# lgleznah/mort

Measured on AMD Instinct MI355X. Metric: Msamples/sec (width x height x spp/s), Scene 1 1200x675, higher is better.
Workload: dtype f32; 1 GPU; Scene 1 (random-spheres cover) 1200x675, 500 spp nominal = 484 effective, depth 20, megakernel, seed 69420, host LCG scene; mode=mega, partition=rows/8 interleaved over 1 rank(s)

## Files before the change

mort_amd/csrc/hip/mega_bvh.h:

```cpp
#ifndef MORT_MEGA_BVH_H
#define MORT_MEGA_BVH_H

#include "dev_render.h"


struct FastArgs {
    RenderArgs r;
    const unsigned char *hot_src;
    uint32_t hot_bytes;
    uint32_t off_nodes4, off_leafrecs, off_lambert, off_metal, off_diel, off_dlight, off_iso, off_solid, off_checker;
    uint32_t off_tstack;
    int node_first, node_count;
    unsigned int *next_q;
    int tiles_x, tiles_total;
    uint32_t off_stack;
    int stack_lds_depth;
    const unsigned *tile_order;
    int gen_tiles;
    int spread_shift;
    unsigned *tile_cost;
    int th_s, th_l, t_keep;
    int sub;
    float *vaccum;
    float4 *deep;
    int prio_tiles, prio_lanes;
    int drain_rounds;
    int tile_key_sum;
    const unsigned *prio_dev;
    int heavy_mod, heavy_num, heavy_cap;
    int lane_cap;
    unsigned long long *wave_log;
};

#ifdef MORT_BVH_PRIVATE_ARGS
#define MORT_BVH_ARG_NAME fa_byval
#else
#define MORT_BVH_ARG_NAME
#endif
#ifdef MORT_BVH_NO_PIN
#define BU_I(x) (x)
#define BU_U(x) (x)
#define BU_F(x) (x)
#define BU_P(x) (x)
#else
#define BU_I(x) uni_i(x)
#define BU_U(x) uni_u(x)
#define BU_F(x) uni_f(x)
#define BU_P(x) uni_p(x)
#endif
__device__ __forceinline__ int uni_i(int x) { return __builtin_amdgcn_readfirstlane(x); }
__device__ __forceinline__ uint32_t uni_u(uint32_t x) { return (uint32_t)__builtin_amdgcn_readfirstlane((int)x); }
__device__ __forceinline__ float uni_f(float x) { return __int_as_float(__builtin_amdgcn_readfirstlane(__float_as_int(x))); }
template <typename T> __device__ __forceinline__ T *uni_p(T *p) {
    const unsigned long long v = (unsigned long long)p;
    const uint32_t lo = uni_u((uint32_t)v), hi = uni_u((uint32_t)(v >> 32));
    return (T *)(((unsigned long long)hi << 32) | (unsigned long long)lo);
}

enum { ST_T = 0, ST_L = 1, ST_S = 2, ST_DONE = 3 };
enum { FL_TIE = 1, FL_REF = 2, FL_MASK = 3 };
#define FL_SIGNS(ox, oy, oz) (int)(((ox) << 8) | ((oy) << 16) | ((oz) << 24))
#ifdef MORT_REGION_MARKS
#define REGION(name) asm volatile("; REGION " name)
#else
#define REGION(name) do { } while (0)
#endif

DEV bool own_inv_ok(float v) { const float a = mort_fabsf(v); return a > 1e-15f && a < 1e15f; }
struct V3Ret { float x, y, z; };
__device__ __attribute__((noinline)) V3Ret texture_value_uv(const DScene *sc, uint32_t tex, float nx, float ny, float nz, float px, float py, float pz) {
    float u, v;
    sphere_uv(mk(nx, ny, nz), u, v);
    const V3 c = texture_value(*sc, tex, u, v, mk(px, py, pz));
    V3Ret r; r.x = c.x; r.y = c.y; r.z = c.z;
    return r;
}

struct RefHit { int best; float closest; };
__device__ __attribute__((noinline)) RefHit reference_walk(const DBvhNode *nodes, int node_first, int node_end, const DSphere *spheres,
                                                           float ox, float oy, float oz, float dx, float dy, float dz, float tm, float ray_a) {
    Ray ray; ray.o = mk(ox, oy, oz); ray.d = mk(dx, dy, dz); ray.tm = tm;
    float closest = __builtin_inff();
    int best = -1;
    const double dix = 1.0 / (double)ray.d.x, diy = 1.0 / (double)ray.d.y, diz = 1.0 / (double)ray.d.z;
    int n = node_first;
    while (n < node_end) {
        const DBvhNode nd = nodes[n];
        const int skip = (int)(nd.skip & 0x7fffffffu);
        if (!slab_exact(nd, ray.o.x, ray.o.y, ray.o.z, dix, diy, diz, closest)) { n = skip; continue; }
        if (!(nd.skip >> 31)) { n = n + 1; continue; }
        const uint32_t pa = nd.prims & 0x7fffu, pb = (nd.prims >> 16) & 0x7fffu;
        for (int k = 0; k < 2; k++) {
            const uint32_t p = k ? pb : pa;
            if (k == 1 && pb == pa) break;
            float t;
            if (sphere_hit_t(spheres[p], ray, ray_a, 0.001f, closest, t)) { closest = t; best = (int)p; }
        }
        n = skip;
    }
    RefHit h; h.best = best; h.closest = closest;
    return h;
}

DEV float sphere_hit_root(const DSphere &s, const Ray &r, float a, float t_min, float t_max) {
    const V3 oc = vsub(r.o, sphere_center(s, r.tm));
    const float half_b = vdot(oc, r.d);
    const float c = vlen2(oc) - s.radius * s.radius;
    const float discriminant = half_b * half_b - a * c;
    if (discriminant < 0) return -1.0f;
    const float sqrtd = mort_sqrtf(discriminant);
    float root = (-half_b - sqrtd) / a;
    if (root < t_min || t_max < root) {
        root = (-half_b + sqrtd) / a;
        if (root < t_min || t_max < root) return -1.0f;
    }
    return root;
}

struct OwnRay { float ix, iy, iz, mx, my, mz, band, invlen; };

DEV bool own_prune(float xmin, float xmax, float ymin, float ymax, float zmin, float zmax, float e, const OwnRay &r, float closest, float &te_out) {
    const float px0 = __builtin_fmaf(xmin, r.ix, -r.mx), px1 = __builtin_fmaf(xmax, r.ix, -r.mx);
    const float py0 = __builtin_fmaf(ymin, r.iy, -r.my), py1 = __builtin_fmaf(ymax, r.iy, -r.my);
    const float pz0 = __builtin_fmaf(zmin, r.iz, -r.mz), pz1 = __builtin_fmaf(zmax, r.iz, -r.mz);
    const float te = __builtin_fmaxf(__builtin_fmaxf(__builtin_fminf(px0, px1), __builtin_fminf(py0, py1)),
                                     __builtin_fmaxf(__builtin_fminf(pz0, pz1), 0.001f));
    const float tx = __builtin_fminf(__builtin_fminf(__builtin_fmaxf(px0, px1), __builtin_fmaxf(py0, py1)), __builtin_fmaxf(pz0, pz1));
    const float tau = __builtin_fmaf(__builtin_fmaxf(mort_fabsf(te), mort_fabsf(tx)), 9.5367431640625e-07f, r.band);
    const float key = __builtin_fmaf(te, 0.992f, -__builtin_fmaf(e, r.invlen, tau));
    te_out = te;
    return (tx - te < -tau) || (key > closest);
}

DEV bool own_prune_ordered(float xn, float xf, float yn, float yf, float zn, float zf, float e, const OwnRay &r, float closest, float &te_out) {
    const float pxn = __builtin_fmaf(xn, r.ix, -r.mx), pxf = __builtin_fmaf(xf, r.ix, -r.mx);
    const float pyn = __builtin_fmaf(yn, r.iy, -r.my), pyf = __builtin_fmaf(yf, r.iy, -r.my);
    const float pzn = __builtin_fmaf(zn, r.iz, -r.mz), pzf = __builtin_fmaf(zf, r.iz, -r.mz);
    const float te = __builtin_fmaxf(__builtin_fmaxf(pxn, pyn), __builtin_fmaxf(pzn, 0.001f));
    const float tx = __builtin_fminf(__builtin_fminf(pxf, pyf), pzf);
    const float tau = __builtin_fmaf(__builtin_fmaxf(mort_fabsf(te), mort_fabsf(tx)), 9.5367431640625e-07f, r.band);
    const float key = __builtin_fmaf(te, 0.992f, -__builtin_fmaf(e, r.invlen, tau));
    te_out = te;
    return (tx - te < -tau) || (key > closest);
}
DEV uint32_t own_sign_offset(float inv) { return (__builtin_bit_cast(uint32_t, inv) >> 27) & 16u; }

typedef float v2f_t __attribute__((ext_vector_type(2)));
DEV void own_prune2(v2f_t xmin, v2f_t xmax, v2f_t ymin, v2f_t ymax, v2f_t zmin, v2f_t zmax, v2f_t e, const OwnRay &r, float closest,
                    float &te_a, float &te_b, bool &skip_a, bool &skip_b) {
    const v2f_t ix = {r.ix, r.ix}, iy = {r.iy, r.iy}, iz = {r.iz, r.iz};
    const v2f_t nmx = {-r.mx, -r.mx}, nmy = {-r.my, -r.my}, nmz = {-r.mz, -r.mz};
    const v2f_t px0 = __builtin_elementwise_fma(xmin, ix, nmx), px1 = __builtin_elementwise_fma(xmax, ix, nmx);
    const v2f_t py0 = __builtin_elementwise_fma(ymin, iy, nmy), py1 = __builtin_elementwise_fma(ymax, iy, nmy);
    const v2f_t pz0 = __builtin_elementwise_fma(zmin, iz, nmz), pz1 = __builtin_elementwise_fma(zmax, iz, nmz);
    v2f_t te, tx;
    te.x = __builtin_fmaxf(__builtin_fmaxf(__builtin_fminf(px0.x, px1.x), __builtin_fminf(py0.x, py1.x)), __builtin_fmaxf(__builtin_fminf(pz0.x, pz1.x), 0.001f));
    te.y = __builtin_fmaxf(__builtin_fmaxf(__builtin_fminf(px0.y, px1.y), __builtin_fminf(py0.y, py1.y)), __builtin_fmaxf(__builtin_fminf(pz0.y, pz1.y), 0.001f));
    tx.x = __builtin_fminf(__builtin_fminf(__builtin_fmaxf(px0.x, px1.x), __builtin_fmaxf(py0.x, py1.x)), __builtin_fmaxf(pz0.x, pz1.x));
    tx.y = __builtin_fminf(__builtin_fminf(__builtin_fmaxf(px0.y, px1.y), __builtin_fmaxf(py0.y, py1.y)), __builtin_fmaxf(pz0.y, pz1.y));
    v2f_t am;
    am.x = __builtin_fmaxf(mort_fabsf(te.x), mort_fabsf(tx.x)); am.y = __builtin_fmaxf(mort_fabsf(te.y), mort_fabsf(tx.y));
    const v2f_t c20 = {9.5367431640625e-07f, 9.5367431640625e-07f}, band = {r.band, r.band}, il = {r.invlen, r.invlen}, c992 = {0.992f, 0.992f};
    const v2f_t tau = __builtin_elementwise_fma(am, c20, band);
    const v2f_t key = __builtin_elementwise_fma(te, c992, -__builtin_elementwise_fma(e, il, tau));
    const v2f_t gap = tx - te;
    te_a = te.x; te_b = te.y;
    skip_a = (gap.x < -tau.x) || (key.x > closest);
    skip_b = (gap.y < -tau.y) || (key.y > closest);
}

// ... 164 lines not shown
            pf.lofs = qx + qly * a.width;
            pf.got = SUB ? 1 + (qly - rly * fa.sub) : 1;
            done = true;
        }
    }
    if (pf.got) {
        const mort_rng_state st = a.states[pf.lofs];
        pf.d = st.d; pf.v0 = st.v[0]; pf.v1 = st.v[1]; pf.v2 = st.v[2]; pf.v3 = st.v[3]; pf.v4 = st.v[4];
    }
    return pf;
}

template <int BLOCK, bool PROBE, bool DRAIN = false, bool SUB = false>
__global__ void __launch_bounds__(BLOCK, BLOCK == 1024 ? 4 : (DRAIN && BLOCK < 768) ? (BLOCK + 255) / 256 : MORT_MIN_WAVES) mega_bvh_kernel(const FastArgs MORT_BVH_ARG_NAME) {
    extern __shared__ __attribute__((aligned(16))) unsigned char lds[];
    __shared__ CamView s_cam;
#ifdef MORT_BVH_PRIVATE_ARGS
    const FastArgs *const fap = &fa_byval;
    const FastArgs &s_fa = fa_byval;
#else
    __shared__ FastArgs s_fa;
    const FastArgs *const fap = (const FastArgs *)__builtin_amdgcn_kernarg_segment_ptr();
    {
        const uint32_t *src = (const uint32_t *)fap;
        uint32_t *dst = (uint32_t *)&s_fa;
        for (uint32_t i = threadIdx.x; i < (uint32_t)(sizeof(FastArgs) / 4); i += BLOCK) dst[i] = src[i];
    }
#endif
    {
        const uint4 *src = (const uint4 *)fap->hot_src;
        uint4 *dst = (uint4 *)lds;
        const uint32_t n16 = fap->hot_bytes >> 4;
        for (uint32_t i = threadIdx.x; i < n16; i += BLOCK) dst[i] = src[i];
    }
    __syncthreads();
    if (threadIdx.x == 0) cam_view_fill(s_cam, s_fa.r);
    __syncthreads();
    const FastArgs &L = s_fa;
    static_assert(sizeof(DNode4) == 16 * MORT_NODE4_PIECES && sizeof(DLeaf2) == 16 * MORT_LEAF2_PIECES, "record strides");
    const float4 *nodes4 = (const float4 *)(lds + BU_U(L.off_nodes4));
    const float4 *leafrecs = (const float4 *)(lds + BU_U(L.off_leafrecs));
    unsigned short *const ts_base = (unsigned short *)(lds + BU_U(L.off_tstack)) + threadIdx.x;
#define TS_AT(ptr) (*(ptr))
    const DLambert *lambert = (const DLambert *)(lds + BU_U(L.off_lambert));
    const DMetal *metal = (const DMetal *)(lds + BU_U(L.off_metal));
    const DDielectric *dielectric = (const DDielectric *)(lds + BU_U(L.off_diel));
    const DLambert *dlight = (const DLambert *)(lds + BU_U(L.off_dlight));
    const DLambert *isotropic = (const DLambert *)(lds + BU_U(L.off_iso));
    const DSolid *solid = (const DSolid *)(lds + BU_U(L.off_solid));
    const DChecker *checker = (const DChecker *)(lds + BU_U(L.off_checker));

    const int node_first = BU_I(L.node_first), node_end = node_first + BU_I(L.node_count);
    const int th_s = BU_I(L.th_s), th_l = BU_I(L.th_l), t_keep = BU_I(L.t_keep);
    const int sqrt_spp = BU_I(L.r.sqrt_spp), bounce_limit = BU_I(L.r.bounce_limit);
    const float bg_x = BU_F(L.r.background.x), bg_y = BU_F(L.r.background.y), bg_z = BU_F(L.r.background.z);
    const int spp = sqrt_spp * sqrt_spp;
    const unsigned total_q = (unsigned)BU_I(L.tiles_total) * 64u;

    int state = ((int)(threadIdx.x & 63u) < BU_I(L.lane_cap)) ? ST_S : ST_DONE, kind = K_NEWPIX;
    int xy = 0, lofs = 0;
    Rng rng; rng.d = rng.v0 = rng.v1 = rng.v2 = rng.v3 = rng.v4 = 0; rng.draws = 0;
    V3 pixel_color = mk(0, 0, 0);
    int s_ij = 0, iter = 0;
    uint32_t segments = 0;
    Ray ray; ray.o = mk(0, 0, 0); ray.d = mk(0, 0, 1); ray.tm = 0;
    float ray_time0 = 0;
    OwnRay orr; orr.ix = orr.iy = orr.iz = 1; orr.mx = orr.my = orr.mz = 0; orr.band = 0; orr.invlen = 1;
    float ray_a = 1, closest = 0;
    int best = -1;
    uint32_t node = 0;
    unsigned short *spa = ts_base;
    int flags = 0;
    float4 *stack_deep = BU_P(L.deep) + ((size_t)blockIdx.x * BLOCK + threadIdx.x);
    const size_t deep_stride = (size_t)gridDim.x * BLOCK;
    unsigned long long ident_mask = 0ull;
    float4 *stack_lds = (float4 *)(lds + BU_U(L.off_stack));
    const int DL = BU_I(L.stack_lds_depth);
#ifdef MORT_PROFILE_STATES
    unsigned long long *const counters_p = fap->r.counters;
    unsigned long long prof[6] = {0, 0, 0, 0, 0, 0};
    unsigned long long prof_truns = 0;
    unsigned long long profc[8] = {0, 0, 0, 0, 0, 0, 0, 0};
    unsigned long long ps0 = 0, ps1;
#define PROFS0() do { ps0 = __builtin_readcyclecounter(); } while (0)
#define PROFS(i) do { ps1 = __builtin_readcyclecounter(); profc[i] += ps1 - ps0; ps0 = ps1; } while (0)
    unsigned long long pt0 = __builtin_readcyclecounter(), pt1;
    const unsigned long long prof_r0 = __builtin_amdgcn_s_memrealtime();
#define PROF(i, lanes) do { prof[2 * (i)] += 1; prof[2 * (i) + 1] += (unsigned long long)(lanes); } while (0)
    unsigned long long profb[12] = {0, 0, 0, 0, 0, 0, 0, 0, 0, 0, 0, 0};
#ifdef MORT_PROFILE_FINE
#define PROFB(i) do { } while (0)
    unsigned long long proff[12] = {0, 0, 0, 0, 0, 0, 0, 0, 0, 0, 0, 0};
#define PROFF(i) do { ps1 = __builtin_readcyclecounter(); proff[i] += ps1 - ps0; profc[4] += ps1 - ps0; ps0 = ps1; } while (0)
#else
#define PROFF(i) do { } while (0)
#define PROFB(i) do { const unsigned long long m_ = __ballot(1); if ((int)(threadIdx.x & 63) == __ffsll((long long)m_) - 1) { \
        atomicAdd(&counters_p[18 + 2 * (i)], 1ull); atomicAdd(&counters_p[19 + 2 * (i)], (unsigned long long)__popcll(m_)); } } while (0)
#endif
#define PROFC(i) do { pt1 = __builtin_readcyclecounter(); profc[i] += pt1 - pt0; pt0 = pt1; } while (0)
#else
#define PROF(i, lanes) do { } while (0)
#define PROFB(i) do { } while (0)
#define PROFF(i) do { } while (0)
#define PROFC(i) do { } while (0)
#define PROFS0() do { } while (0)
#define PROFS(i) do { } while (0)
#endif

    int leader = -1;
    const bool drain_rounds = DRAIN && BU_I(L.drain_rounds) == 1;
    const bool live_thresholds = BU_I(L.drain_rounds) == 3;
    bool running = true;
    while (running) {
      int nS = 0;
      for (;;) {
        const unsigned long long mT = __ballot(state == ST_T);
        const unsigned long long mL = __ballot(state == ST_L);
        const unsigned long long mS = __ballot(state == ST_S);
        if ((mT | mL | mS) == 0ull) { running = false; break; }
        const int nT = __popcll(mT), nL = __popcll(mL);
        nS = __popcll(mS);
        int pick;
        int e_s = th_s, e_l = th_l;
        if (live_thresholds) { const int live = nT + nL + nS; e_s = (th_s * live + 63) >> 6; e_l = (th_l * live + 63) >> 6; }
        if (nS >= e_s) pick = ST_S;
        else if (nL >= e_l) pick = ST_L;
        else if (nT > 0) pick = ST_T;
        else pick = (nL >= nS) ? ST_L : ST_S;
        if (DRAIN && leader >= 0) {
            if (drain_rounds) pick = nT > 0 ? ST_T : nL > 0 ? ST_L : ST_S;
            else { const int ls = __builtin_amdgcn_readlane(state, leader); if (ls <= ST_S) pick = ls; }
        }
        PROFC(3);

                REGION("T");
        if (pick != ST_T && pick != ST_L) break;
        if (pick == ST_T) {
            int keep;
#ifdef MORT_PROFILE_STATES
            prof_truns++;
#endif
            do {
#pragma unroll
                for (int rep = 0; rep < MORT_T_UNROLL; rep++) {
                PROF(0, __popcll(__ballot(state == ST_T)));
                if (state == ST_T) {
                    const float4 *np = nodes4 + node;
                    float t0, t1, t2, t3;
#ifdef MORT_BVH_PACKED_FMA
                    const float4 bx0 = np[MORT_NODE4_X], bx1 = np[MORT_NODE4_X + 1], by0 = np[MORT_NODE4_Y], by1 = np[MORT_NODE4_Y + 1];
                    const float4 bz0 = np[MORT_NODE4_Z], bz1 = np[MORT_NODE4_Z + 1], be = np[MORT_NODE4_E];
                    const uint4 ch = ((const uint4 *)np)[MORT_NODE4_CHILD];
                    bool m0, m1, m2, m3;
                    own_prune2(v2f_t{bx0.x, bx0.y}, v2f_t{bx1.x, bx1.y}, v2f_t{by0.x, by0.y}, v2f_t{by1.x, by1.y}, v2f_t{bz0.x, bz0.y}, v2f_t{bz1.x, bz1.y}, v2f_t{be.x, be.y}, orr, closest, t0, t1, m0, m1);
                    own_prune2(v2f_t{bx0.z, bx0.w}, v2f_t{bx1.z, bx1.w}, v2f_t{by0.z, by0.w}, v2f_t{by1.z, by1.w}, v2f_t{bz0.z, bz0.w}, v2f_t{bz1.z, bz1.w}, v2f_t{be.z, be.w}, orr, closest, t2, t3, m2, m3);
                    m2 = m2 || ch.z == 0xffffu; m3 = m3 || ch.w == 0xffffu;
#else
                    const unsigned char *nb = (const unsigned char *)np;
                    const float4 *ax = (const float4 *)(nb + (((uint32_t)flags >> 8) & 0xffu)) + MORT_NODE4_X;
                    const float4 *ay = (const float4 *)(nb + (((uint32_t)flags >> 16) & 0xffu)) + MORT_NODE4_Y;
                    const float4 *az = (const float4 *)(nb + ((uint32_t)flags >> 24)) + MORT_NODE4_Z;
                    const float4 xn = ax[0], xf = ax[1], yn = ay[0], yf = ay[1], zn = az[0], zf = az[1], be = np[MORT_NODE4_E];
                    const uint4 ch = ((const uint4 *)np)[MORT_NODE4_CHILD];
                    const bool m0 = own_prune_ordered(xn.x, xf.x, yn.x, yf.x, zn.x, zf.x, be.x, orr, closest, t0);
                    const bool m1 = own_prune_ordered(xn.y, xf.y, yn.y, yf.y, zn.y, zf.y, be.y, orr, closest, t1);
                    const bool m2 = own_prune_ordered(xn.z, xf.z, yn.z, yf.z, zn.z, zf.z, be.z, orr, closest, t2) || ch.z == 0xffffu;
                    const bool m3 = own_prune_ordered(xn.w, xf.w, yn.w, yf.w, zn.w, zf.w, be.w, orr, closest, t3) || ch.w == 0xffffu;
#endif
                    uint32_t k0 = m0 ? 0xffffffffu : ((__float_as_uint(t0) & 0xffff0000u) | ch.x);
                    uint32_t k1 = m1 ? 0xffffffffu : ((__float_as_uint(t1) & 0xffff0000u) | ch.y);
                    uint32_t k2 = m2 ? 0xffffffffu : ((__float_as_uint(t2) & 0xffff0000u) | ch.z);
                    uint32_t k3 = m3 ? 0xffffffffu : ((__float_as_uint(t3) & 0xffff0000u) | ch.w);
#define MORT_CSWAP(a, b) do { const uint32_t lo_ = a < b ? a : b, hi_ = a < b ? b : a; a = lo_; b = hi_; } while (0)
                    MORT_CSWAP(k0, k1); MORT_CSWAP(k2, k3); MORT_CSWAP(k0, k2); MORT_CSWAP(k1, k3); MORT_CSWAP(k1, k2);
#undef MORT_CSWAP
#ifdef MORT_BVH_PUSH_BRANCHFREE
                    TS_AT(spa) = (unsigned short)k3; spa += (k3 != 0xffffffffu) ? BLOCK : 0;
                    TS_AT(spa) = (unsigned short)k2; spa += (k2 != 0xffffffffu) ? BLOCK : 0;
                    TS_AT(spa) = (unsigned short)k1; spa += (k1 != 0xffffffffu) ? BLOCK : 0;
#else
                    if (k3 != 0xffffffffu) { TS_AT(spa) = (unsigned short)k3; spa += BLOCK; }
                    if (k2 != 0xffffffffu) { TS_AT(spa) = (unsigned short)k2; spa += BLOCK; }
                    if (k1 != 0xffffffffu) { TS_AT(spa) = (unsigned short)k1; spa += BLOCK; }
#endif
                    uint32_t next = k0;
                    const bool none = k0 == 0xffffffffu;
                    const bool have = !none || spa != ts_base;
                    if (none && spa != ts_base) { spa -= BLOCK; next = TS_AT(spa); }
                    if (!have) { state = ST_S; kind = K_SHADE; }
                    else { node = next & 0x7fffu; if (next & 0x8000u) state = ST_L; }
                }
                }
                keep = __popcll(__ballot(state == ST_T));
                if (DRAIN && leader >= 0) keep = drain_rounds ? (keep > 0 ? 64 : 0) : (__builtin_amdgcn_readlane(state, leader) == ST_T) ? 64 : 0;
                else if (keep > 0 && keep < t_keep) {
                    const int wL = __popcll(__ballot(state == ST_L)), wS = __popcll(__ballot(state == ST_S));
                    if (!(wS >= e_s || wL >= e_l)) keep = 64;
                }
            } while (keep >= t_keep);
            PROFC(0);
        }
        if (pick == ST_L) {
                REGION("L");
            PROF(1, nL);
            if (state == ST_L) {
                const float4 *lp = leafrecs + node;
                const float4 a0 = lp[0], a1 = lp[1], b0 = lp[2], b1 = lp[3];
                const uint32_t two = ((const uint4 *)lp)[5].z;
                DSphere sa, sb;
                sa.cx = a0.x; sa.cy = a0.y; sa.cz = a0.z; sa.radius = a0.w; sa.vx = a1.x; sa.vy = a1.y; sa.vz = a1.z; sa.mat = __float_as_uint(a1.w);
                sb.cx = b0.x; sb.cy = b0.y; sb.cz = b0.z; sb.radius = b0.w; sb.vx = b1.x; sb.vy = b1.y; sb.vz = b1.z; sb.mat = __float_as_uint(b1.w);
                const float ta = sphere_hit_root(sa, ray, ray_a, 0.001f, closest);
                if (ta != -1.0f) {
                    if (ta == closest && best >= 0) flags |= FL_TIE;
                    closest = ta; best = (int)(node << 16);
                }
                if (two == 2u) {
                    const float tb = sphere_hit_root(sb, ray, ray_a, 0.001f, closest);
                    if (tb != -1.0f) {
                        if (tb == closest && best >= 0) flags |= FL_TIE;
                        closest = tb; best = (int)((node << 16) | 0x8000u);
                    }
                }
                if (spa != ts_base) {
                    spa -= BLOCK;
                    const uint32_t next = TS_AT(spa);
                    node = next & 0x7fffu;
                    state = (next & 0x8000u) ? ST_L : ST_T;
                } else { state = ST_S; kind = K_SHADE; }
            }
            PROFC(1);
        }
      }
      if (!running) break;
        {
            PROF(2, nS);
            PROFS0();
            V3 final_value = mk(0, 0, 0);
                REGION("S:verify");
            if (state == ST_S) {
                if (kind == K_SHADE) {
                    bool need_ref = (flags & FL_MASK) != 0;
                    if (!need_ref && best >= 0) {
                        const float4 *lp = leafrecs + (best >> 16);
                        const float4 b0 = lp[4], b1 = lp[5];
                        DBvhNode lb;
                        lb.xmin = b0.x; lb.xmax = b0.y; lb.ymin = b0.z; lb.ymax = b0.w; lb.zmin = b1.x; lb.zmax = b1.y; lb.skip = 0; lb.prims = 0;
                        need_ref = !slab_check(lb, ray, orr, closest);
                    }
                    if (need_ref) {
                        atomicAdd(&fap->r.counters[3], 1ull);
                        const RefHit h = reference_walk(fap->r.sc.nodes, node_first, node_end, fap->r.sc.spheres, ray.o.x, ray.o.y, ray.o.z,
                                                        ray.d.x, ray.d.y, ray.d.z, ray.tm, ray_a);
                        best = h.best; closest = h.closest;
                    }
                    PROFF(0);
                REGION("S:hitrecord");
                    if (best < 0) {
                        final_value = mk(bg_x, bg_y, bg_z);
                        kind = K_FINISH;
                    } else {
                        DSphere sp;
                        if (need_ref) sp = fap->r.sc.spheres[best];
                        else {
                            const float4 *lp = leafrecs + (best >> 16) + ((best & 0x8000) ? 2 : 0);
                            const float4 s0 = lp[0], s1 = lp[1];
                            sp.cx = s0.x; sp.cy = s0.y; sp.cz = s0.z; sp.radius = s0.w; sp.vx = s1.x; sp.vy = s1.y; sp.vz = s1.z; sp.mat = __float_as_uint(s1.w);
                        }
                        const V3 p = ray_at(ray, closest);
                        const V3 outward = vdiv(vsub(p, sphere_center(sp, ray.tm)), sp.radius);
                        const bool front_face = vdot(ray.d, outward) < 0;
                        const V3 normal = front_face ? outward : vneg(outward);
                        const int mtype = DREF_TYPE(sp.mat), midx = DREF_IDX(sp.mat);
                        PROFF(1);
                        StackEntry e;
                        if (mtype == MORT_MAT_METAL) {
                REGION("S:metal");
// ... 113 lines not shown
                    ident_mask = 0ull;
                    pixel_color = vadd(pixel_color, final_value);
                    s_ij++;
                    bool more;
                    if constexpr (SUB) {
                        more = (s_ij & 0xffff) != sqrt_spp;
                    } else {
                        if ((s_ij & 0xffff) == sqrt_spp) s_ij = (s_ij & ~0xffff) + 0x10000;
                        more = (s_ij >> 16) < sqrt_spp;
                    }
                    if (more) {
                        kind = K_NEWSAMPLE;
                    } else {
                        pixel_write<PROBE, SUB>(fap, pixel_color.x, pixel_color.y, pixel_color.z, lofs, segments, rng.draws, rng.d, rng.v0, rng.v1, rng.v2, rng.v3, rng.v4);
                        kind = K_NEWPIX;
                    }
                }
                REGION("S:newpix");
                PROFS(5);
                if (kind == K_NEWPIX) {
                    const PixelFetch pf = pixel_fetch<SUB>(fap, total_q);
                    if (!pf.got) state = ST_DONE;
                    else {
                        xy = pf.xy; lofs = pf.lofs;
                        rng.d = pf.d; rng.v0 = pf.v0; rng.v1 = pf.v1; rng.v2 = pf.v2; rng.v3 = pf.v3; rng.v4 = pf.v4;
                        rng.draws = 0;
                        pixel_color = mk(0, 0, 0);
                        s_ij = SUB ? ((pf.got - 1) << 16) : 0; segments = 0;
                        kind = (spp > 0) ? K_NEWSAMPLE : K_FINISH;
                        if (spp <= 0) {
                            final_value = mk(0, 0, 0);
                        }
                    }
                }
                REGION("S:getray");
                PROFS(6);
                if (state != ST_DONE) {
                    if (kind == K_NEWSAMPLE) {
                        PROFB(4);
                        ray = get_ray(s_cam, xy & 0xffff, (xy >> 16) & 0x7fff, rng, s_ij & 0xffff, s_ij >> 16);
                        ray_time0 = ray.tm;
                        iter = 0;
                        kind = K_SHADE;
                        if (bounce_limit <= 0) { final_value = mk(0, 0, 0); kind = K_FINISH; }
                    }
                REGION("S:setup");
                    if (kind == K_SHADE) {
                        ray_a = vlen2(ray.d);
                        orr.ix = 1.0f / ray.d.x; orr.iy = 1.0f / ray.d.y; orr.iz = 1.0f / ray.d.z;
                        orr.mx = ray.o.x * orr.ix; orr.my = ray.o.y * orr.iy; orr.mz = ray.o.z * orr.iz;
                        const float mm = __builtin_fmaxf(__builtin_fmaxf(mort_fabsf(orr.mx), mort_fabsf(orr.my)), mort_fabsf(orr.mz));
                        orr.band = mm * 4.76837158203125e-07f;
                        orr.invlen = 1.01f / mort_sqrtf(ray_a);
                        const bool ordinary = own_inv_ok(orr.ix) && own_inv_ok(orr.iy) && own_inv_ok(orr.iz) && (mm < 1e30f);
                        closest = __builtin_inff();
                        best = -1;
                        node = 0; spa = ts_base;
                        flags = ordinary ? FL_SIGNS(own_sign_offset(orr.ix), own_sign_offset(orr.iy), own_sign_offset(orr.iz)) : FL_REF;
                        segments++;
                        state = ordinary ? ST_T : ST_S;
                    }
                }
            }
                REGION("S:end");
            if (DRAIN && __ballot(state == ST_DONE) != 0ull) {
                unsigned key = (state <= ST_S) ? ((unsigned)((s_ij >> 16) * sqrt_spp + (s_ij & 0xffff)) << 6) | (threadIdx.x & 63u) : 0xffffffffu;
                for (int off = 32; off > 0; off >>= 1) { const unsigned o = (unsigned)__shfl_xor((int)key, off); key = o < key ? o : key; }
                leader = (key == 0xffffffffu) ? -1 : __builtin_amdgcn_readfirstlane((int)(key & 63u));
            }
            PROFS(7);
            PROFC(2);
        }
    }
    if ((threadIdx.x & 63) == 0) {
#ifdef MORT_PROFILE_STATES
#ifdef MORT_PROFILE_FINE
        for (int k = 0; k < 12; k++) atomicAdd(&counters_p[18 + k], proff[k]);
#endif
        for (int k = 0; k < 6; k++) atomicAdd(&counters_p[4 + k], prof[k]);
        atomicAdd(&counters_p[30], prof_truns);
        for (int k = 0; k < 4; k++) atomicAdd(&counters_p[10 + k], profc[k]);
        for (int k = 4; k < 8; k++) atomicAdd(&counters_p[14 + k - 4], profc[k]);
        if (fap->wave_log) {
            unsigned long long *w = fap->wave_log + 16 * ((size_t)blockIdx.x * (BLOCK / 64) + (threadIdx.x >> 6));
            w[0] = blockIdx.x; w[1] = threadIdx.x >> 6; w[2] = __builtin_amdgcn_s_memrealtime() - prof_r0;
            w[3] = prof[0]; w[4] = prof[2]; w[5] = 0; w[6] = prof[4]; w[7] = profc[0]; w[8] = profc[1]; w[9] = 0; w[10] = profc[2]; w[11] = profc[3];
        }
        (void)profb;
#endif
    }
}

#endif
```

mort_amd/csrc/hip/mort_hip.hip:

```cpp
#include <hip/hip_runtime.h>

#include <algorithm>
#include <array>
#include <climits>
#include <cmath>
#include <cstdio>
#include <cstdlib>
#include <cstring>
#include <new>
#include <string>
#include <thread>
#include <vector>

#include "mort_hip.h"
#include "dev_pixel.h"
#include "scene_blob.h"
#include "seed_host.h"
#include "mort_internal.h"
#include "mort_ctx.h"
#include "mega_gen.h"
#include "wave_gen.h"

#pragma clang fp contract(off)

// ... 546 lines not shown
    if (std::getenv("MORT_WAVE_LINES")) {
        c->wave_log_waves = (size_t)grid * (size_t)(FB / 64);
        if (ensure_buf(c, &c->d_wave_log, &c->wave_log_cap, c->wave_log_waves * 16 * sizeof(unsigned long long)) == MORT_OK) {
            hipMemsetAsync(c->d_wave_log, 0, c->wave_log_waves * 16 * sizeof(unsigned long long), s);
            fa.wave_log = (unsigned long long *)c->d_wave_log;
        }
    }
    return MORT_OK;
}

typedef void (*bvh_kernel_t)(const FastArgs);
static bvh_kernel_t bvh_kernel(int FB, bool probe, bool drain, bool sub) {
    if (!sub) switch (FB) {
        case 1024: return !probe ? mega_bvh_kernel<1024, false, false> : mega_bvh_kernel<1024, true, false>;
        case 768: return probe ? mega_bvh_kernel<768, true, false> : drain ? mega_bvh_kernel<768, false, true> : mega_bvh_kernel<768, false, false>;
        case 512: return probe ? mega_bvh_kernel<512, true, false> : drain ? mega_bvh_kernel<512, false, true> : mega_bvh_kernel<512, false, false>;
        case 384: return probe ? mega_bvh_kernel<384, true, false> : drain ? mega_bvh_kernel<384, false, true> : mega_bvh_kernel<384, false, false>;
        default: return probe ? mega_bvh_kernel<256, true, false> : drain ? mega_bvh_kernel<256, false, true> : mega_bvh_kernel<256, false, false>;
    }
    return FB == 1024 ? mega_bvh_kernel<1024, false, false, true> : FB == 768 ? mega_bvh_kernel<768, false, false, true> : FB == 512 ? mega_bvh_kernel<512, false, false, true>
           : FB == 384 ? mega_bvh_kernel<384, false, false, true> : mega_bvh_kernel<256, false, false, true>;
}

static int launch_bvh(mort_ctx *c, const mort_camera *cam, const RenderArgs &a, int tiles, bool sub, bool timed, hipStream_t s, LaunchPlan &plan) {
    FastArgs fa;
    std::memset(&fa, 0, sizeof fa);
    fast_args_base(c, cam, a, fa, c->d_fast, c->fast_bytes, tiles, sub);
    fa.off_nodes4 = c->f_nodes4; fa.off_leafrecs = c->f_leafrecs; fa.off_lambert = c->f_lambert; fa.off_metal = c->f_metal;
    fa.off_diel = c->f_diel; fa.off_dlight = c->f_dlight; fa.off_iso = c->f_iso; fa.off_solid = c->f_solid; fa.off_checker = c->f_checker;
    fa.node_first = 0; fa.node_count = c->sc.n_nodes;
    const long long lanes_wanted = (long long)tiles * 64;
    const double px_per_lane = (double)lanes_wanted / ((double)c->num_cus * 768.0);
    int FB = MORT_FAST_BLOCK;
    const char *fb_env = std::getenv("MORT_FAST_BLOCK_SIZE");
    if (fb_env) FB = std::atoi(fb_env);
    else {
        const int cand[4] = {768, 512, 384, 256};
        FB = 256;
        const bool wide_ok = lanes_wanted >= 2ll * 1024 * c->num_cus;
        for (int k = (px_per_lane < 1.5 && !sub) ? 1 : 0; k < 4; k++) if (lanes_wanted >= (long long)cand[k] * c->num_cus) { FB = cand[k]; break; }
        if (wide_ok) FB = 1024;
    }
    if (FB == 1024 && !bvh_wide_block_fits(fa.hot_bytes, c->own4_stack)) FB = 768;
    if (FB != 1024 && FB != 768 && FB != 512 && FB != 384) FB = 256;
    fa.drain_rounds = 3;
    { const char *dm = std::getenv("MORT_BVH_DRAIN"); if (dm) fa.drain_rounds = std::atoi(dm) == 2 ? 1 : std::atoi(dm) == 3 ? 3 : 0; }
    bool chain_bound = px_per_lane < 1.5 && !sub;
    { const char *cb = std::getenv("MORT_CHAIN_BOUND"); if (cb && !sub) chain_bound = cb[0] == '1'; }
    if (FB == 1024) chain_bound = false;
    const bvh_kernel_t kern = bvh_kernel(FB, false, chain_bound, sub), kern_probe = bvh_kernel(FB, true, false, false);
    fa.th_s = MORT_TH_S; fa.th_l = MORT_TH_L; fa.t_keep = MORT_T_KEEP;
    { const char *th = std::getenv("MORT_THRESHOLDS");
      if (th) { int s_ = 0, l_ = 0, k_ = 0; if (std::sscanf(th, "%d,%d,%d", &s_, &l_, &k_) == 3 && s_ >= 1 && l_ >= 1 && k_ >= 1) { fa.th_s = s_; fa.th_l = l_; fa.t_keep = k_; } } }
    int per_cu_cap = INT_MAX;
    { const char *pc = std::getenv("MORT_FAST_BLOCKS_PER_CU"); if (pc && std::atoi(pc) >= 1) per_cu_cap = std::atoi(pc); }
    size_t lds_bytes = 0;
    int grid = 0;
    int st = state_setup(c, cam, fa, (const void *)kern, FB, (uint32_t)c->own4_stack + MORT_BVH_TSTACK_SPARE, 12, per_cu_cap, "BVH image does not fit one CU's LDS", s, lds_bytes, grid);
    if (st != MORT_OK) return st;
    st = prepare_tile_order(c, cam, a, fa, tiles, grid, FB, chain_bound, sub, timed, s, [&](const FastArgs &pa) {
        hipError_t e_ = hipFuncSetAttribute((const void *)kern_probe, hipFuncAttributeMaxDynamicSharedMemorySize, (int)lds_bytes);
        if (e_ != hipSuccess) return e_;
        hipLaunchKernelGGL(kern_probe, dim3(grid), dim3(FB), lds_bytes, s, pa);
        return hipGetLastError();
    });
    if (st != MORT_OK) return st;
    hipLaunchKernelGGL(kern, dim3(grid), dim3(FB), lds_bytes, s, fa);
    HIPCHK(c, hipGetLastError());
    plan.kernel = (const void *)kern; plan.block = FB; plan.lds_bytes = (int)lds_bytes;
    std::snprintf(plan.name, sizeof plan.name, "mega_bvh_kernel<%d, false, %s, %s>", FB, chain_bound ? "true" : "false", sub ? "true" : "false");
    return MORT_OK;
}

static int launch_gen(mort_ctx *c, const mort_camera *cam, const RenderArgs &a, int tiles, bool sub, bool timed, hipStream_t s, LaunchPlan &plan) {
    GenArgs ga = c->gen;
    FastArgs &fa = ga.f;
    fast_args_base(c, cam, a, fa, c->d_gen, c->gen_bytes, tiles, sub);
    const long long lanes_wanted = (long long)tiles * 64;
    int FB = 768;
    bool heavy_default = false;
    { const char *fb_env = std::getenv("MORT_GEN_BLOCK_SIZE");
      if (fb_env && !sub) FB = std::atoi(fb_env);
      else {
             const double ppl = (double)lanes_wanted / ((double)c->num_cus * 768.0);
             FB = ppl >= 8.0 ? 1024 : (lanes_wanted >= 512ll * c->num_cus) ? 512 : 256;
             if (ppl < 8.0 && lanes_wanted >= 32ll * 1024 && !std::getenv("MORT_GEN_NO_HEAVY")) { FB = 1024; heavy_default = true; } } }
    if (FB != 1024 && FB != 768 && FB != 512 && FB != 256) FB = 256;
    if (FB == 1024 && (size_t)c->gen_bytes + 16u + (size_t)MORT_OWN_STACK * 1024u * 2u + 2048u > 160u * 1024u) FB = 768;
    if (sub && FB > 512) FB = 512;
    fa.th_s = 28; fa.th_l = 20; fa.t_keep = 4; ga.th_m = 56;
    fa.heavy_mod = 0; fa.heavy_num = 0; fa.heavy_cap = 64; c->heavy_percent = 50;
    if (heavy_default && FB == 1024 && !sub) { fa.heavy_mod = 3; fa.heavy_num = 2; fa.heavy_cap = 12; }
    { const char *hv = std::getenv("MORT_GEN_HEAVY"); int m_ = 0, n_ = 0, k_ = 0, p_ = 0;
      if (hv && !sub && std::sscanf(hv, "%d,%d,%d,%d", &m_, &n_, &k_, &p_) == 4 && m_ >= 1 && n_ >= 1 && n_ <= m_ && k_ >= 1 && k_ <= 64 && p_ >= 1 && p_ <= 100) {
          fa.heavy_mod = m_; fa.heavy_num = n_; fa.heavy_cap = k_; c->heavy_percent = p_; } }
    ga.drain_mode = 3;
    { const char *dm = std::getenv("MORT_GEN_DRAIN"); if (dm && std::atoi(dm) >= 0 && std::atoi(dm) <= 3) ga.drain_mode = std::atoi(dm); }
    { const char *th = std::getenv("MORT_GEN_THRESHOLDS");
      if (th) { int s_ = 0, l_ = 0, k_ = 0, m_ = 0; if (std::sscanf(th, "%d,%d,%d,%d", &s_, &l_, &k_, &m_) == 4 && s_ >= 1 && l_ >= 1 && k_ >= 1 && m_ >= 1) { fa.th_s = s_; fa.th_l = l_; fa.t_keep = k_; ga.th_m = m_; } } }
    const gen_kernel_t kern = mort_gen_kernel(FB, ga.prims_in_lds != 0, sub);
    int dl_cap = 12;
    { const char *de = std::getenv("MORT_GEN_DL"); if (de) dl_cap = std::atoi(de) > 0 ? std::atoi(de) : 0; }
    size_t lds_bytes = 0;
    int grid = 0;
    int st = state_setup(c, cam, fa, (const void *)kern, FB, MORT_OWN_STACK, dl_cap, INT_MAX, "unified-tree image does not fit one CU's LDS", s, lds_bytes, grid);
    if (st != MORT_OK) return st;
// ... 303 lines not shown
    if (st != MORT_OK) return st;
    const std::vector<DNode4> &nodes = sb.comp.own_nodes4;
    for (int i = 0; i < 16; i++) out[i] = 0;
    out[4] = nodes.size();
    if (nodes.empty()) return MORT_OK;
    for (const DNode4 &nd : nodes)
        for (int k = 0; k < 4; k++) {
            if (nd.child[k] != 0xffffu) continue;
            const float v[10] = {nd.x[0][k], nd.x[1][k], nd.x[2][k], nd.y[0][k], nd.y[1][k], nd.y[2][k], nd.z[0][k], nd.z[1][k], nd.z[2][k], nd.e[k]};
            for (float f : v) { uint32_t b; std::memcpy(&b, &f, 4); if (b) { out[5]++; break; } }
        }
    unsigned nthreads = std::thread::hardware_concurrency();
    if (nthreads < 1) nthreads = 1;
    if (nthreads > 16) nthreads = 16;
    std::vector<std::array<unsigned long long, 16>> part(nthreads);
    auto work = [&](unsigned t) {
        std::array<unsigned long long, 16> &o = part[t];
        o.fill(0);
        for (size_t r = t; r < n; r += nthreads) {
            const float *q = rays + 7 * r;
            OwnRay orr;
            orr.ix = 1.0f / q[3]; orr.iy = 1.0f / q[4]; orr.iz = 1.0f / q[5];
            orr.mx = q[0] * orr.ix; orr.my = q[1] * orr.iy; orr.mz = q[2] * orr.iz;
            const float mm = __builtin_fmaxf(__builtin_fmaxf(mort_fabsf(orr.mx), mort_fabsf(orr.my)), mort_fabsf(orr.mz));
            orr.band = mm * 4.76837158203125e-07f;
            orr.invlen = 1.01f / mort_sqrtf(q[3] * q[3] + q[4] * q[4] + q[5] * q[5]);
            if (!(own_inv_ok(orr.ix) && own_inv_ok(orr.iy) && own_inv_ok(orr.iz) && (mm < 1e30f))) { o[3]++; continue; }
            const uint32_t sx = own_sign_offset(orr.ix) / 16u, sy = own_sign_offset(orr.iy) / 16u, sz = own_sign_offset(orr.iz) / 16u;
            o[8 + (sx | sy << 1 | sz << 2)]++;
            const float closest = q[6];
            for (size_t ni = r % (size_t)stride; ni < nodes.size(); ni += (size_t)stride) {
                const DNode4 &nd = nodes[ni];
                for (int k = 0; k < 4; k++) {
                    if (nd.child[k] == 0xffffu) continue;
                    float te_a, te_b;
                    const bool skip_a = own_prune(nd.x[0][k], nd.x[1][k], nd.y[0][k], nd.y[1][k], nd.z[0][k], nd.z[1][k], nd.e[k], orr, closest, te_a);
                    const bool skip_b = own_prune_ordered(nd.x[sx][k], nd.x[sx + 1][k], nd.y[sy][k], nd.y[sy + 1][k], nd.z[sz][k], nd.z[sz + 1][k], nd.e[k], orr, closest, te_b);
                    o[0]++;
                    if (std::memcmp(&te_a, &te_b, 4) != 0) o[1]++;
                    if (skip_a != skip_b) o[2]++;
                    if (skip_a && skip_b) o[6]++;
                }
            }
        }
    };
    std::vector<std::thread> pool;
    for (unsigned t = 1; t < nthreads; t++) pool.emplace_back(work, t);
    work(0);
    for (std::thread &th : pool) th.join();
    for (const auto &o : part) for (int i = 0; i < 16; i++) if (i != 4 && i != 5) out[i] += o[i];
    return MORT_OK;
}

extern "C" int mort_hip_render_device(mort_ctx *c, const mort_camera *cam, int mode, void *d_rgba, void *d_accum,
                                      void *stream, mort_stats *stats) {
    return render_device_impl(c, cam, mode, d_rgba, d_accum, nullptr, stream, stats);
}

extern "C" int mort_hip_render(mort_ctx *c, const mort_camera *cam, int mode, uint8_t *rgba_out, float *accum_out,
                               uint32_t *segments_px_out, mort_stats *stats) {
    if (!c || !cam || !rgba_out) return MORT_ERR_INVALID;
    const int W = cam->image_width, H = cam->image_height;
    if (W <= 0 || H <= 0) return MORT_ERR_INVALID;
    HIPCHK(c, hipSetDevice(c->device));
    const int lr = local_rows_for(c->part, H);
    const size_t npx = (size_t)W * (size_t)lr;
    int st;
    if ((st = ensure_buf(c, &c->d_rgba, &c->rgba_cap, npx * 4)) != MORT_OK) return st;
    if (accum_out && (st = ensure_buf(c, &c->d_accum, &c->accum_cap, npx * 12)) != MORT_OK) return st;
    if (segments_px_out) { if ((st = ensure_buf(c, &c->d_segpx, &c->segpx_cap, npx * 4)) != MORT_OK) return st; }
    else if (c->d_segpx) { hipFree(c->d_segpx); c->d_segpx = nullptr; c->segpx_cap = 0; }
    mort_stats local;
    st = render_device_impl(c, cam, mode, c->d_rgba, accum_out ? c->d_accum : nullptr,
                            segments_px_out ? (uint32_t *)c->d_segpx : nullptr, nullptr, &local);
    if (st != MORT_OK) return st;
    if (stats) *stats = local;
    if (c->part.nranks == 1) {
        HIPCHK(c, hipMemcpy(rgba_out, c->d_rgba, npx * 4, hipMemcpyDeviceToHost));
        if (accum_out) HIPCHK(c, hipMemcpy(accum_out, c->d_accum, npx * 12, hipMemcpyDeviceToHost));
        if (segments_px_out) HIPCHK(c, hipMemcpy(segments_px_out, c->d_segpx, npx * 4, hipMemcpyDeviceToHost));
        return MORT_OK;
    }
    for (int ly = 0; ly < lr; ly++) {
        const int y = global_row_host(c->part, ly);
        HIPCHK(c, hipMemcpy(rgba_out + (size_t)y * W * 4, (uint8_t *)c->d_rgba + (size_t)ly * W * 4, (size_t)W * 4, hipMemcpyDeviceToHost));
        if (accum_out) HIPCHK(c, hipMemcpy(accum_out + (size_t)y * W * 3, (float *)c->d_accum + (size_t)ly * W * 3, (size_t)W * 12, hipMemcpyDeviceToHost));
        if (segments_px_out) HIPCHK(c, hipMemcpy(segments_px_out + (size_t)y * W, (uint32_t *)c->d_segpx + (size_t)ly * W, (size_t)W * 4, hipMemcpyDeviceToHost));
    }
    return MORT_OK;
}
```

Baseline: 4232 Msamples/s.

## Split leaf sphere test into wave-uniform root loop and add deferred-leaf option

The two-sphere leaf test now computes both discriminants up front. It then runs the sqrt/divide root block in a loop of at most two trips that exits once no lane in the wave has a pending hit, so lanes do not wait through a divergent second root computation. An opt-in mode (MORT_BVH_DEFER, off by default) holds one leaf in the upper bits of the node register during traversal, so leaf visits can be batched. The change also fixes tie-flag handling via tie_update, adds a NaN check on the ray offsets, and adds a host-side debug walker that compares the leaf forms. The default kernel path changes its leaf code and adds masking on node indices, which may cost extra instructions in the hot loop.

```diff
diff --git a/mort_amd/csrc/hip/mega_bvh.h b/mort_amd/csrc/hip/mega_bvh.h
--- a/mort_amd/csrc/hip/mega_bvh.h
+++ b/mort_amd/csrc/hip/mega_bvh.h
@@ -30,6 +30,7 @@
     int heavy_mod, heavy_num, heavy_cap;
     int lane_cap;
     unsigned long long *wave_log;
+    int defer_leaf;
 };
 
 #ifdef MORT_BVH_PRIVATE_ARGS
@@ -102,12 +103,16 @@
     return h;
 }
 
-DEV float sphere_hit_root(const DSphere &s, const Ray &r, float a, float t_min, float t_max) {
+struct SphereHalf { float half_b, discriminant; };
+DEV SphereHalf sphere_hit_half(const DSphere &s, const Ray &r, float a) {
     const V3 oc = vsub(r.o, sphere_center(s, r.tm));
-    const float half_b = vdot(oc, r.d);
+    SphereHalf h;
+    h.half_b = vdot(oc, r.d);
     const float c = vlen2(oc) - s.radius * s.radius;
-    const float discriminant = half_b * half_b - a * c;
-    if (discriminant < 0) return -1.0f;
+    h.discriminant = h.half_b * h.half_b - a * c;
+    return h;
+}
+DEV float sphere_root_block(float half_b, float discriminant, float a, float t_min, float t_max) {
     const float sqrtd = mort_sqrtf(discriminant);
     float root = (-half_b - sqrtd) / a;
     if (root < t_min || t_max < root) {
@@ -116,6 +121,20 @@
     }
     return root;
 }
+DEV float sphere_hit_root(const DSphere &s, const Ray &r, float a, float t_min, float t_max) {
+    const SphereHalf h = sphere_hit_half(s, r, a);
+    if (h.discriminant < 0) return -1.0f;
+    return sphere_root_block(h.half_b, h.discriminant, a, t_min, t_max);
+}
+
+DEV int tie_update(int flags, float t, float closest, int best) {
+    return (t < closest) ? (flags & ~FL_TIE) : (best >= 0) ? (flags | FL_TIE) : flags;
+}
+
+#define NODE_AT(n) ((n) & 0x7fffu)
+#define NODE_HELD(n) ((int)(n) < 0)
+#define NODE_HELD_LEAF(n) (((n) >> 16) & 0x7fffu)
+#define NODE_HOLD(n, ref) ((n) | ((ref) << 16))
 
 struct OwnRay { float ix, iy, iz, mx, my, mz, band, invlen; };
 
@@ -386,6 +405,7 @@
 
     const int node_first = BU_I(L.node_first), node_end = node_first + BU_I(L.node_count);
     const int th_s = BU_I(L.th_s), th_l = BU_I(L.th_l), t_keep = BU_I(L.t_keep);
+    const bool defer = BU_I(L.defer_leaf) != 0;
     const int sqrt_spp = BU_I(L.r.sqrt_spp), bounce_limit = BU_I(L.r.bounce_limit);
     const float bg_x = BU_F(L.r.background.x), bg_y = BU_F(L.r.background.y), bg_z = BU_F(L.r.background.z);
     const int spp = sqrt_spp * sqrt_spp;
@@ -479,7 +499,7 @@
                 for (int rep = 0; rep < MORT_T_UNROLL; rep++) {
                 PROF(0, __popcll(__ballot(state == ST_T)));
                 if (state == ST_T) {
-                    const float4 *np = nodes4 + node;
+                    const float4 *np = nodes4 + NODE_AT(node);
                     float t0, t1, t2, t3;
 #ifdef MORT_BVH_PACKED_FMA
                     const float4 bx0 = np[MORT_NODE4_X], bx1 = np[MORT_NODE4_X + 1], by0 = np[MORT_NODE4_Y], by1 = np[MORT_NODE4_Y + 1];
@@ -519,10 +539,15 @@
 #endif
                     uint32_t next = k0;
                     const bool none = k0 == 0xffffffffu;
-                    const bool have = !none || spa != ts_base;
                     if (none && spa != ts_base) { spa -= BLOCK; next = TS_AT(spa); }
-                    if (!have) { state = ST_S; kind = K_SHADE; }
-                    else { node = next & 0x7fffu; if (next & 0x8000u) state = ST_L; }
+                    if (defer) {
+                        if ((next & 0x8000u) && !NODE_HELD(node) && spa != ts_base) {
+                            node = NODE_HOLD(node, next);
+                            spa -= BLOCK; next = TS_AT(spa);
+                        } else if (next == 0xffffffffu && NODE_HELD(node)) { next = node >> 16; node = 0; }
+                    }
+                    if (next == 0xffffffffu) { state = ST_S; kind = K_SHADE; }
+                    else { node = (node & 0xffff0000u) | (next & 0x7fffu); if (next & 0x8000u) state = ST_L; }
                 }
                 }
                 keep = __popcll(__ballot(state == ST_T));
@@ -538,25 +563,46 @@
                 REGION("L");
             PROF(1, nL);
             if (state == ST_L) {
-                const float4 *lp = leafrecs + node;
+                const float4 *lp = leafrecs + NODE_AT(node);
                 const float4 a0 = lp[0], a1 = lp[1], b0 = lp[2], b1 = lp[3];
                 const uint32_t two = ((const uint4 *)lp)[5].z;
                 DSphere sa, sb;
                 sa.cx = a0.x; sa.cy = a0.y; sa.cz = a0.z; sa.radius = a0.w; sa.vx = a1.x; sa.vy = a1.y; sa.vz = a1.z; sa.mat = __float_as_uint(a1.w);
                 sb.cx = b0.x; sb.cy = b0.y; sb.cz = b0.z; sb.radius = b0.w; sb.vx = b1.x; sb.vy = b1.y; sb.vz = b1.z; sb.mat = __float_as_uint(b1.w);
+#ifdef MORT_BVH_LEAF_SEQUENTIAL
                 const float ta = sphere_hit_root(sa, ray, ray_a, 0.001f, closest);
                 if (ta != -1.0f) {
-                    if (ta == closest && best >= 0) flags |= FL_TIE;
+                    flags = tie_update(flags, ta, closest, best);
                     closest = ta; best = (int)(node << 16);
                 }
                 if (two == 2u) {
                     const float tb = sphere_hit_root(sb, ray, ray_a, 0.001f, closest);
                     if (tb != -1.0f) {
-                        if (tb == closest && best >= 0) flags |= FL_TIE;
+                        flags = tie_update(flags, tb, closest, best);
                         closest = tb; best = (int)((node << 16) | 0x8000u);
                     }
                 }
-                if (spa != ts_base) {
+#else
+                const SphereHalf ha = sphere_hit_half(sa, ray, ray_a);
+                SphereHalf hb; hb.half_b = 0.0f; hb.discriminant = -1.0f;
+                if (two == 2u) hb = sphere_hit_half(sb, ray, ray_a);
+                uint32_t todo = (!(ha.discriminant < 0) ? 1u : 0u) | ((two == 2u && !(hb.discriminant < 0)) ? 2u : 0u);
+#pragma nounroll
+                for (int trip = 0; trip < 2; trip++) {
+                    if (__ballot(todo != 0u) == 0ull) break;
+                    if (todo != 0u) {
+                        const bool second = !(todo & 1u);
+                        const float t = sphere_root_block(second ? hb.half_b : ha.half_b, second ? hb.discriminant : ha.discriminant, ray_a, 0.001f, closest);
+                        if (t != -1.0f) {
+                            flags = tie_update(flags, t, closest, best);
+                            closest = t; best = (int)((node << 16) | (second ? 0x8000u : 0u));
+                        }
+                        todo &= todo - 1u;
+                    }
+                }
+#endif
+                if (NODE_HELD(node)) node = NODE_HELD_LEAF(node);
+                else if (spa != ts_base) {
                     spa -= BLOCK;
                     const uint32_t next = TS_AT(spa);
                     node = next & 0x7fffu;
@@ -776,7 +822,8 @@
                         const float mm = __builtin_fmaxf(__builtin_fmaxf(mort_fabsf(orr.mx), mort_fabsf(orr.my)), mort_fabsf(orr.mz));
                         orr.band = mm * 4.76837158203125e-07f;
                         orr.invlen = 1.01f / mort_sqrtf(ray_a);
-                        const bool ordinary = own_inv_ok(orr.ix) && own_inv_ok(orr.iy) && own_inv_ok(orr.iz) && (mm < 1e30f);
+                        const float msum = orr.mx + orr.my + orr.mz;
+                        const bool ordinary = own_inv_ok(orr.ix) && own_inv_ok(orr.iy) && own_inv_ok(orr.iz) && (mm < 1e30f) && (msum == msum);
                         closest = __builtin_inff();
                         best = -1;
                         node = 0; spa = ts_base;
diff --git a/mort_amd/csrc/hip/mort_hip.hip b/mort_amd/csrc/hip/mort_hip.hip
--- a/mort_amd/csrc/hip/mort_hip.hip
+++ b/mort_amd/csrc/hip/mort_hip.hip
@@ -622,6 +622,8 @@
     fa.th_s = MORT_TH_S; fa.th_l = MORT_TH_L; fa.t_keep = MORT_T_KEEP;
     { const char *th = std::getenv("MORT_THRESHOLDS");
       if (th) { int s_ = 0, l_ = 0, k_ = 0; if (std::sscanf(th, "%d,%d,%d", &s_, &l_, &k_) == 3 && s_ >= 1 && l_ >= 1 && k_ >= 1) { fa.th_s = s_; fa.th_l = l_; fa.t_keep = k_; } } }
+    fa.defer_leaf = 0;
+    { const char *df = std::getenv("MORT_BVH_DEFER"); if (df && (df[0] == '0' || df[0] == '1') && !df[1]) fa.defer_leaf = df[0] - '0'; }
     int per_cu_cap = INT_MAX;
     { const char *pc = std::getenv("MORT_FAST_BLOCKS_PER_CU"); if (pc && std::atoi(pc) >= 1) per_cu_cap = std::atoi(pc); }
     size_t lds_bytes = 0;
@@ -1031,6 +1033,149 @@
     return MORT_OK;
 }
 
+struct LeafWalk { uint32_t box_steps, leaf_visits, trips, best, closest_bits, flags, stack_max, ended; };
+static void leaf_forms_walk(const std::vector<DNode4> &nodes, const std::vector<DLeaf2> &recs, const float *q, bool loop, bool defer, LeafWalk &o) {
+    enum { STACK_CAP = 64 };
+    Ray ray; ray.o = mk(q[0], q[1], q[2]); ray.d = mk(q[3], q[4], q[5]); ray.tm = q[6];
+    const float ray_a = vlen2(ray.d);
+    OwnRay orr;
+    orr.ix = 1.0f / ray.d.x; orr.iy = 1.0f / ray.d.y; orr.iz = 1.0f / ray.d.z;
+    orr.mx = ray.o.x * orr.ix; orr.my = ray.o.y * orr.iy; orr.mz = ray.o.z * orr.iz;
+    const float mm = __builtin_fmaxf(__builtin_fmaxf(mort_fabsf(orr.mx), mort_fabsf(orr.my)), mort_fabsf(orr.mz));
+    orr.band = mm * 4.76837158203125e-07f;
+    orr.invlen = 1.01f / mort_sqrtf(ray_a);
+    const float msum = orr.mx + orr.my + orr.mz;
+    const bool ordinary = own_inv_ok(orr.ix) && own_inv_ok(orr.iy) && own_inv_ok(orr.iz) && (mm < 1e30f) && (msum == msum);
+    float closest = __builtin_inff();
+    int best = -1;
+    uint32_t node = 0;
+    int flags = ordinary ? 0 : FL_REF;
+    int state = ordinary ? ST_T : ST_S;
+    uint16_t stack[STACK_CAP];
+    uint32_t sp = 0;
+    std::memset(&o, 0, sizeof o);
+    o.ended = 1;
+    const uint32_t sx = own_sign_offset(orr.ix) / 16u, sy = own_sign_offset(orr.iy) / 16u, sz = own_sign_offset(orr.iz) / 16u;
+    const uint64_t step_cap = 8 * (uint64_t)(nodes.size() + recs.size()) + 16;
+    uint64_t steps = 0;
+    while (state != ST_S) {
+        if (++steps > step_cap) { o.ended = 0; break; }
+        if (state == ST_T) {
+            const uint32_t at = NODE_AT(node);
+            if (at % MORT_NODE4_PIECES || at / MORT_NODE4_PIECES >= nodes.size()) { o.ended = 0; break; }
+            const DNode4 &nd = nodes[at / MORT_NODE4_PIECES];
+            o.box_steps++;
+            uint32_t k[4];
+            for (int c = 0; c < 4; c++) {
+                float te;
+                bool m = own_prune_ordered(nd.x[sx][c], nd.x[sx + 1][c], nd.y[sy][c], nd.y[sy + 1][c], nd.z[sz][c], nd.z[sz + 1][c], nd.e[c], orr, closest, te);
+                if (c >= 2) m = m || nd.child[c] == 0xffffu;
+                uint32_t tb; std::memcpy(&tb, &te, 4);
+                k[c] = m ? 0xffffffffu : ((tb & 0xffff0000u) | nd.child[c]);
+            }
+#define LF_CSWAP(a, b) do { const uint32_t lo_ = a < b ? a : b, hi_ = a < b ? b : a; a = lo_; b = hi_; } while (0)
+            LF_CSWAP(k[0], k[1]); LF_CSWAP(k[2], k[3]); LF_CSWAP(k[0], k[2]); LF_CSWAP(k[1], k[3]); LF_CSWAP(k[1], k[2]);
+#undef LF_CSWAP
+            bool overflow = false;
+            for (int c = 3; c >= 1; c--) if (k[c] != 0xffffffffu) { if (sp >= STACK_CAP) { overflow = true; break; } stack[sp++] = (uint16_t)k[c]; }
+            if (overflow) { o.ended = 0; o.stack_max = STACK_CAP + 1; break; }
+            if (sp > o.stack_max) o.stack_max = sp;
+            uint32_t next = k[0];
+            const bool none = k[0] == 0xffffffffu;
+            if (none && sp != 0) next = stack[--sp];
+            if (defer) {
+                if ((next & 0x8000u) && !NODE_HELD(node) && sp != 0) {
+                    node = NODE_HOLD(node, next);
+                    next = stack[--sp];
+                } else if (next == 0xffffffffu && NODE_HELD(node)) { next = node >> 16; node = 0; }
+            }
+            if (next == 0xffffffffu) state = ST_S;
+            else { node = (node & 0xffff0000u) | (next & 0x7fffu); if (next & 0x8000u) state = ST_L; }
+        } else {
+            const uint32_t at = NODE_AT(node);
+            if (at % MORT_LEAF2_PIECES || at / MORT_LEAF2_PIECES >= recs.size()) { o.ended = 0; break; }
+            const DLeaf2 &lr = recs[at / MORT_LEAF2_PIECES];
+            o.leaf_visits++;
+            const uint32_t two = lr.n;
+            if (!loop) {
+                const SphereHalf ha = sphere_hit_half(lr.a, ray, ray_a);
+                const float ta = sphere_hit_root(lr.a, ray, ray_a, 0.001f, closest);
+                if (!(ha.discriminant < 0)) o.trips++;
+                if (ta != -1.0f) {
+                    flags = tie_update(flags, ta, closest, best);
+                    closest = ta; best = (int)(node << 16);
+                }
+                if (two == 2u) {
+                    const SphereHalf hb = sphere_hit_half(lr.b, ray, ray_a);
+                    const float tb = sphere_hit_root(lr.b, ray, ray_a, 0.001f, closest);
+                    if (!(hb.discriminant < 0)) o.trips++;
+                    if (tb != -1.0f) {
+                        flags = tie_update(flags, tb, closest, best);
+                        closest = tb; best = (int)((node << 16) | 0x8000u);
+                    }
+                }
+            } else {
+                const SphereHalf ha = sphere_hit_half(lr.a, ray, ray_a);
+                SphereHalf hb; hb.half_b = 0.0f; hb.discriminant = -1.0f;
+                if (two == 2u) hb = sphere_hit_half(lr.b, ray, ray_a);
+                uint32_t todo = (!(ha.discriminant < 0) ? 1u : 0u) | ((two == 2u && !(hb.discriminant < 0)) ? 2u : 0u);
+                uint32_t trips_here = 0;
+                for (int trip = 0; trip < 2; trip++) {
+                    if (todo == 0u) break;
+                    trips_here++;
+                    const bool second = !(todo & 1u);
+                    const float t = sphere_root_block(second ? hb.half_b : ha.half_b, second ? hb.discriminant : ha.discriminant, ray_a, 0.001f, closest);
+                    if (t != -1.0f) {
+                        flags = tie_update(flags, t, closest, best);
+                        closest = t; best = (int)((node << 16) | (second ? 0x8000u : 0u));
+                    }
+                    todo &= todo - 1u;
+                }
+                if (todo != 0u) { o.ended = 0; break; }
+                o.trips += trips_here;
+            }
+            if (NODE_HELD(node)) node = NODE_HELD_LEAF(node);
+            else if (sp != 0) {
+                const uint32_t next = stack[--sp];
+                node = next & 0x7fffu;
+                state = (next & 0x8000u) ? ST_L : ST_T;
+            } else state = ST_S;
+        }
+    }
+    if (o.ended && (NODE_HELD(node) || sp != 0)) o.ended = 0;
+    if (flags & FL_MASK) best = -2;
+    o.best = (uint32_t)best; std::memcpy(&o.closest_bits, &closest, 4); o.flags = (uint32_t)(flags & FL_MASK);
+}
+
+extern "C" int mort_hip_debug_leaf_forms(const mort_world *w, const float *rays, size_t n, uint32_t *out, int *info) {
+    if (!w || (!rays && n) || (!out && n) || !info) return MORT_ERR_INVALID;
+    SceneBlob sb;
+    const int st = build_scene_blob(w, sb);
+    if (st != MORT_OK) return st;
+    const std::vector<DNode4> &nodes = sb.comp.own_nodes4;
+    const std::vector<DLeaf2> &recs = sb.comp.own_leafrecs;
+    info[0] = (int)nodes.size(); info[1] = (int)recs.size(); info[2] = sb.comp.own4_stack; info[3] = 0;
+    for (const DLeaf2 &r : recs) if (r.n == 2u) info[3]++;
+    if (nodes.empty()) return MORT_OK;
+    static_assert(sizeof(LeafWalk) == 32, "eight words per form");
+    unsigned nthreads = std::thread::hardware_concurrency();
+    if (nthreads < 1) nthreads = 1;
+    if (nthreads > 16) nthreads = 16;
+    auto work = [&](unsigned t) {
+        for (size_t r = t; r < n; r += nthreads)
+            for (int form = 0; form < 4; form++) {
+                LeafWalk lw;
+                leaf_forms_walk(nodes, recs, rays + 7 * r, (form & 1) != 0, (form & 2) != 0, lw);
+                std::memcpy(out + (r * 4 + (size_t)form) * 8, &lw, sizeof lw);
+            }
+    };
+    std::vector<std::thread> pool;
+    for (unsigned t = 1; t < nthreads; t++) pool.emplace_back(work, t);
+    work(0);
+    for (std::thread &th : pool) th.join();
+    return MORT_OK;
+}
+
 extern "C" int mort_hip_render_device(mort_ctx *c, const mort_camera *cam, int mode, void *d_rgba, void *d_accum,
                                       void *stream, mort_stats *stats) {
     return render_device_impl(c, cam, mode, d_rgba, d_accum, nullptr, stream, stats);
```

After: 4122 Msamples/s. -2.6%, worse.
